# 3DOM-FBK/deep-image-matching

Measured on NVIDIA H100. Metric: image-pairs/sec (SuperPoint+LightGlue, 1024x1024, 2048 kpts), higher is better.
Workload: dtype f16 hi/lo split x3 MMA, f32 accumulate (fp32-class)

## Files before the change

deep-image-matching_b200/csrc/gemm.cuh:

```cuda
#pragma once
#include "common.cuh"
#include "sm90.cuh"

struct TileCoord {
  int m0;
  int n0;
  int b, y0, x0;
};

struct GemmArgs {
  int num_kb;
  int k_total;
  int M;
  int N;
  int cin_blocks;
  int H, W;
  int tiles_x, tiles_y;
  const __half *Ah, *Al, *Bh, *Bl;
  int lda, ldb;
};

constexpr int kTileM = 128;
constexpr int kGemmThreads = 12 * 32;
constexpr int kProducerRegs = 40, kConsumerRegs = 232;
constexpr int kScratchPitch = 32;
constexpr int kScratchFloats = 32 * kScratchPitch;
constexpr int kStgCols = 64, kStgPitch = kStgCols + 4;
constexpr int kStgFloats = 64 * kStgPitch;
constexpr int kStgBytes = 2 * kStgFloats * 4;
static_assert(4 * kScratchFloats <= kStgFloats, "functor scratch must fit in the staging buffer of a warpgroup");
constexpr int kConvTH = 8, kConvTW = 16;
template <int CONV>
struct ConvTile {
  static constexpr int TH = kConvTH, TW = kConvTW;
};

template <int CONV>
__device__ __forceinline__ TileCoord make_tile_coord(const GemmArgs& g, int t) {
  TileCoord tc;
  if (CONV == 1) {
    int per_img = g.tiles_x * g.tiles_y;
    tc.b = t / per_img;
    int rem = t - tc.b * per_img;
    tc.y0 = (rem / g.tiles_x) * ConvTile<CONV>::TH;
    tc.x0 = (rem % g.tiles_x) * ConvTile<CONV>::TW;
    tc.m0 = 0;
    tc.n0 = 0;
  } else {
    tc.m0 = t * kTileM;
    tc.n0 = 0;
    tc.b = tc.y0 = tc.x0 = 0;
  }
  return tc;
}

struct PersCfg {
  int sa, sb;
  int nkb_total;
  int smem_bytes;
};

template <int BN, bool SPLIT, int CONV>
struct PersGeom {
  static constexpr int kPl = SPLIT ? 2 : 1;
  static constexpr int kRowB = CONV == 3 ? 64 : 128;
  static constexpr int kABoxTx = CONV == 1 ? (kConvTH + 2) * kConvTW * 128 : kTileM * kRowB;
  static constexpr int kABox = (kABoxTx + 1023) / 1024 * 1024;
  static constexpr int kATx = kPl * kABoxTx;
  static constexpr int kAStage = kPl * kABox;
  static constexpr int kBPlane = BN * kRowB;
  static constexpr int kBTile = kPl * kBPlane;
  static constexpr int kBudget = 232448 - 1024 - 1024 - kStgBytes;
};

template <int BN, bool SPLIT, int CONV, bool RESB, class Epi>
__global__ void __launch_bounds__(kGemmThreads, 1)
tc_gemm_pers_kernel(const __grid_constant__ CUtensorMap tmAh, const __grid_constant__ CUtensorMap tmAl,
                    const __grid_constant__ CUtensorMap tmBh, const __grid_constant__ CUtensorMap tmBl, GemmArgs g, Epi epi,
                    int m_tiles, int n_tiles, int SA, int SB) {
  using G = PersGeom<BN, SPLIT, CONV>;
  using namespace sm90;
  static_assert(BN % kStgCols == 0, "BN must be a multiple of the staging width");
  extern __shared__ uint8_t smem_raw[];
  uint8_t* smem = smem_raw + ((1024u - (sm90::smem_u32(smem_raw) & 1023u)) & 1023u);
  constexpr bool ISCONV = CONV == 1;
  constexpr bool K32 = CONV == 3;
  constexpr int KB_COLS = K32 ? 32 : 64;
  constexpr int KSTEPS = K32 ? 2 : 4;
  constexpr uint32_t kLayout = K32 ? kLayoutSw64 : kLayoutSw128;
  constexpr uint32_t kSbo = 8 * G::kRowB;
  const int nkb = g.num_kb;
  uint8_t* sA = smem;
  uint8_t* sB = sA + SA * G::kAStage;
  const int nb_slots = RESB ? nkb : SB;
  uint64_t* fullA = reinterpret_cast<uint64_t*>(sB + nb_slots * G::kBTile);
  uint64_t* emptyA = fullA + SA;
  uint64_t* fullB = emptyA + SA;
  uint64_t* emptyB = fullB + nb_slots;
  float* staging = reinterpret_cast<float*>(reinterpret_cast<uint8_t*>(fullA) + 1024);

  const int warp = threadIdx.x >> 5, lane = threadIdx.x & 31;
  if (threadIdx.x == 0) {
    for (int s = 0; s < SA; ++s) {
      mbar_init(&fullA[s], 1);
      mbar_init(&emptyA[s], 8);
    }
    for (int s = 0; s < nb_slots; ++s) {
      mbar_init(&fullB[s], 1);
      mbar_init(&emptyB[s], 8);
    }
    fence_barrier_init();
  }
  __syncthreads();
  const int total = m_tiles * n_tiles;
  const int cinb = ISCONV ? g.cin_blocks : 1;
  const int outer_n = ISCONV ? 3 * cinb : nkb;
  constexpr int inner_n = ISCONV ? 3 : 1;
  auto kb_of = [&](int o, int in) { return ISCONV ? ((in * 3 + o / cinb) * cinb + (o % cinb)) : o; };

  auto tile_coord = [&](int w, int& n0) {
    const int mt = w / n_tiles, nt = w - mt * n_tiles;
    TileCoord tc = make_tile_coord<CONV>(g, mt);
    if (!ISCONV) tc.m0 = epi.m0_of(mt);
    n0 = nt * BN;
    tc.n0 = n0;
    return tc;
  };

  if (warp >= 8) {
    setmaxnreg_dec<kProducerRegs>();
    if (warp == 8) {
      if (elect_one()) {
        tma_prefetch_desc(&tmAh);
        tma_prefetch_desc(&tmBh);
        if (SPLIT) {
          tma_prefetch_desc(&tmAl);
          tma_prefetch_desc(&tmBl);
        }
      }
      __syncwarp();
      if (RESB && elect_one()) {
        const int nres = (static_cast<int>(blockIdx.x) % n_tiles) * BN;
        for (int kb = 0; kb < nkb; ++kb) {
          mbar_expect_tx(&fullB[kb], G::kBTile);
          tma_load_2d(sB + kb * G::kBTile, &tmBh, &fullB[kb], kb * KB_COLS, nres);
          if (SPLIT) tma_load_2d(sB + kb * G::kBTile + G::kBPlane, &tmBl, &fullB[kb], kb * KB_COLS, nres);
        }
      }
      __syncwarp();
      uint32_t itA = 0, itB = 0;
      for (int w = blockIdx.x; w < total; w += gridDim.x) {
        int n0;
        const TileCoord tc = tile_coord(w, n0);
        if (!epi.tile_active(tc)) continue;
        const int b_off = epi.b_row_offset(tc);
        const int outer = outer_n;
        if (elect_one()) {
          const int wp = w + 2 * static_cast<int>(gridDim.x);
          if (wp < total) {
            int n0p;
            const TileCoord tp = tile_coord(wp, n0p);
            if ((ISCONV || n0p == 0) && epi.tile_active(tp)) {
              for (int o = 0; o < outer; ++o) {
                if (ISCONV) {
                  const int dx = o / cinb, cb = o - dx * cinb;
                  if (dx != 1) continue;
                  tma_prefetch_4d(&tmAh, cb * 64, tp.x0 - 1, tp.y0 - 1, tp.b);
                  if (SPLIT) tma_prefetch_4d(&tmAl, cb * 64, tp.x0 - 1, tp.y0 - 1, tp.b);
                  tma_prefetch_4d(&tmAh, cb * 64, tp.x0 + 1, tp.y0 - 1, tp.b);
                  if (SPLIT) tma_prefetch_4d(&tmAl, cb * 64, tp.x0 + 1, tp.y0 - 1, tp.b);
                } else {
                  tma_prefetch_2d(&tmAh, o * KB_COLS, tp.m0);
                  if (SPLIT) tma_prefetch_2d(&tmAl, o * KB_COLS, tp.m0);
                }
              }
            }
          }
        }
        __syncwarp();
        for (int o = 0; o < outer; ++o) {
          const int s = itA % SA;
          mbar_wait(&emptyA[s], ((itA / SA) & 1) ^ 1);
          uint8_t* st = sA + s * G::kAStage;
          if (elect_one()) {
            mbar_expect_tx(&fullA[s], G::kATx);
            if (ISCONV) {
              const int dx = o / cinb, cb = o - dx * cinb;
              tma_load_4d(st, &tmAh, &fullA[s], cb * 64, tc.x0 + dx - 1, tc.y0 - 1, tc.b);
              if (SPLIT) tma_load_4d(st + G::kABox, &tmAl, &fullA[s], cb * 64, tc.x0 + dx - 1, tc.y0 - 1, tc.b);
            } else {
              tma_load_2d(st, &tmAh, &fullA[s], o * KB_COLS, tc.m0);
              if (SPLIT) tma_load_2d(st + G::kABox, &tmAl, &fullA[s], o * KB_COLS, tc.m0);
            }
          }
          __syncwarp();
          ++itA;
          if (!RESB) {
            for (int dy = 0; dy < inner_n; ++dy) {
              const int kb = kb_of(o, dy);
              const int sb = itB % SB;
              mbar_wait(&emptyB[sb], ((itB / SB) & 1) ^ 1);
              uint8_t* bt = sB + sb * G::kBTile;
              if (elect_one()) {
                mbar_expect_tx(&fullB[sb], G::kBTile);
                tma_load_2d(bt, &tmBh, &fullB[sb], kb * KB_COLS, n0 + b_off);
                if (SPLIT) tma_load_2d(bt + G::kBPlane, &tmBl, &fullB[sb], kb * KB_COLS, n0 + b_off);
              }
              __syncwarp();
              ++itB;
            }
          }
        }
      }
    }
  } else {
    setmaxnreg_inc<kConsumerRegs>();
    const int wg = warp >> 2, w4 = warp & 3;
    const uint32_t a_wg = static_cast<uint32_t>(wg * 64 * G::kRowB);
    float* stg = staging + wg * kStgFloats;
    uint32_t itA = 0, itB = 0;
    bool resb_ready = false;
    float acc[BN / 2];
    for (int w = blockIdx.x; w < total; w += gridDim.x) {
      int n0;
      const TileCoord tc = tile_coord(w, n0);
      if (!epi.tile_active(tc)) continue;
      const int outer = outer_n;
      for (int o = 0; o < outer; ++o) {
        const int s = itA % SA;
        mbar_wait(&fullA[s], (itA / SA) & 1);
        const uint32_t a_base = smem_u32(sA + s * G::kAStage) + a_wg;
        int sb0 = 0;
#pragma unroll
        for (int dy = 0; dy < inner_n; ++dy) {
          const int kb = kb_of(o, dy);
          uint32_t b_base;
          if (RESB) {
            if (!resb_ready) mbar_wait(&fullB[kb], 0);
            b_base = smem_u32(sB + kb * G::kBTile);
          } else {
            const int sb = (itB + dy) % SB;
            if (dy == 0) sb0 = sb;
            mbar_wait(&fullB[sb], ((itB + dy) / SB) & 1);
            b_base = smem_u32(sB + sb * G::kBTile);
          }
          const uint32_t a_tap = a_base + (ISCONV ? dy * (kConvTW * 128) : 0);
          const uint64_t a_h = make_sdesc(a_tap, kSbo, kLayout), a_l = make_sdesc(a_tap + G::kABox, kSbo, kLayout);
          const uint64_t b_h = make_sdesc(b_base, kSbo, kLayout), b_l = make_sdesc(b_base + G::kBPlane, kSbo, kLayout);
          wgmma_fence();
#pragma unroll
          for (int k16 = 0; k16 < KSTEPS; ++k16) {
            Wgmma<BN>::ss(acc, sdesc_advance_k(a_h, k16), sdesc_advance_k(b_h, k16), (o | dy | k16) != 0);
            if (SPLIT) {
              Wgmma<BN>::ss(acc, sdesc_advance_k(a_h, k16), sdesc_advance_k(b_l, k16), 1);
              Wgmma<BN>::ss(acc, sdesc_advance_k(a_l, k16), sdesc_advance_k(b_h, k16), 1);
            }
          }
        }
        wgmma_commit();
        wgmma_wait<0>();
        wgmma_fence_regs(acc);
        if (lane == 0) {
          mbar_arrive(&emptyA[s]);
          if (!RESB)
            for (int dy = 0; dy < inner_n; ++dy) mbar_arrive(&emptyB[(sb0 + dy) % SB]);
        }
        ++itA;
        if (!RESB) itB += inner_n;
      }
      resb_ready = true;
      const int rr = 32 * (w4 & 1) + lane, cq = 32 * (w4 >> 1);
#pragma unroll
      for (int c0 = 0; c0 < BN; c0 += kStgCols) {
        const int lr = 16 * w4 + (lane >> 2);
#pragma unroll
        for (int i = c0 / 8; i < (c0 + kStgCols) / 8; ++i) {
          const int col = 8 * i - c0 + 2 * (lane & 3);
          *reinterpret_cast<float2*>(stg + lr * kStgPitch + col) = make_float2(acc[4 * i], acc[4 * i + 1]);
          *reinterpret_cast<float2*>(stg + (lr + 8) * kStgPitch + col) = make_float2(acc[4 * i + 2], acc[4 * i + 3]);
        }
        named_bar_sync(1 + wg, 128);
        float v[32];
#pragma unroll
        for (int q = 0; q < 8; ++q) {
          const float4 x = *reinterpret_cast<const float4*>(stg + rr * kStgPitch + cq + 4 * q);
          v[4 * q] = x.x, v[4 * q + 1] = x.y, v[4 * q + 2] = x.z, v[4 * q + 3] = x.w;
        }
        named_bar_sync(1 + wg, 128);
        epi(tc, 64 * wg + rr, n0 + c0 + cq, v, stg + w4 * kScratchFloats);
        named_bar_sync(1 + wg, 128);
      }
    }
    if (RESB && !resb_ready)
      for (int kb = 0; kb < nkb; ++kb) mbar_wait(&fullB[kb], 0);
  }
}

template <int CONV>
__device__ __forceinline__ float simt_load_a(const GemmArgs& g, const TileCoord& tc, int row, int k) {
  size_t off;
  if (CONV == 1) {
    const int cin = g.cin_blocks * 64;
    const int tap = k / cin, c = k - tap * cin;
    const int dy = tap / 3, dx = tap - dy * 3;
    const int y = tc.y0 + row / ConvTile<CONV>::TW + dy - 1, x = tc.x0 + row % ConvTile<CONV>::TW + dx - 1;
    if (y < 0 || y >= g.H || x < 0 || x >= g.W) return 0.f;
    off = ((static_cast<size_t>(tc.b) * g.H + y) * g.W + x) * cin + c;
  } else {
    const int gm = tc.m0 + row;
    if (gm >= g.M) return 0.f;
    off = static_cast<size_t>(gm) * g.lda + k;
  }
  float v = __half2float(g.Ah[off]);
  if (g.Al) v += __half2float(g.Al[off]);
  return v;
}

template <int CONV, class Epi>
__global__ void __launch_bounds__(128) simt_gemm_kernel(GemmArgs g, Epi epi) {
  TileCoord tc = make_tile_coord<CONV>(g, blockIdx.x);
  if (CONV != 1) tc.m0 = epi.m0_of(blockIdx.x);
  tc.n0 = blockIdx.y * 32;
  if (!epi.tile_active(tc)) return;
  const int b_off = epi.b_row_offset(tc);
  __shared__ float As[128][33];
  __shared__ float Bs[32][33];
  __shared__ __align__(16) float scratchS[4 * kScratchFloats];
  const int t = threadIdx.x, n0 = blockIdx.y * 32;
  float acc[32];
#pragma unroll
  for (int j = 0; j < 32; ++j) acc[j] = 0.f;
  const int K = g.k_total ? g.k_total : g.num_kb * 64;
  for (int k0 = 0; k0 < K; k0 += 32) {
    const int kk = t & 31;
    for (int i = 0; i < 32; ++i) {
      const int row = i * 4 + (t >> 5);
      As[row][kk] = simt_load_a<CONV>(g, tc, row, k0 + kk);
    }
    for (int i = 0; i < 8; ++i) {
      const int nn = i * 4 + (t >> 5);
      float b = 0.f;
      if (n0 + nn < g.N) {
        const size_t off = static_cast<size_t>(n0 + nn + b_off) * g.ldb + k0 + kk;
        b = __half2float(g.Bh[off]);
        if (g.Bl) b += __half2float(g.Bl[off]);
      }
      Bs[nn][kk] = b;
    }
    __syncthreads();
#pragma unroll 4
    for (int k = 0; k < 32; ++k) {
      const float a = As[t][k];
#pragma unroll
      for (int j = 0; j < 32; ++j) acc[j] = fmaf(a, Bs[j][k], acc[j]);
    }
    __syncthreads();
  }
  epi(tc, t, n0, acc, scratchS + (t >> 5) * kScratchFloats);
}

struct TcOperands {
  CUtensorMap Ah, Al, Bh, Bl;
};

template <int BN, bool SPLIT, int CONV, bool RESB, class Epi>
int launch_pers(dimb_ctx* ctx, cudaStream_t st, const TcOperands& ops, const GemmArgs& g, const Epi& epi, int m_tiles, int n_tiles,
                const PersCfg& cfg, int grid) {
  auto kern = tc_gemm_pers_kernel<BN, SPLIT, CONV, RESB, Epi>;
  DIMB_TRY(dimb_func_smem(ctx, kern, cfg.smem_bytes));
  kern<<<grid, kGemmThreads, cfg.smem_bytes, st>>>(ops.Ah, ops.Al, ops.Bh, ops.Bl, g, epi, m_tiles, n_tiles, cfg.sa, cfg.sb);
  DIMB_LAUNCH_CHECK(ctx);
  return DIMB_OK;
}

template <int BN, bool SPLIT, int CONV>
PersCfg pers_config(int nkb, bool resb) {
  using G = PersGeom<BN, SPLIT, CONV>;
  PersCfg c{};
  c.nkb_total = nkb;
  int budget = G::kBudget;
  if (resb) {
    budget -= nkb * G::kBTile;
    c.sb = 0;
    c.sa = budget / G::kAStage;
  } else {
    const int per = CONV == 1 ? 3 : 1;
    const int unit = G::kAStage + per * G::kBTile;
    int n = budget / unit;
    if (n < 1) n = 1;
    c.sa = n;
    c.sb = per * n;
    while (c.sa * G::kAStage + (c.sb + 1) * G::kBTile <= budget) ++c.sb;
    while ((c.sa + 1) * G::kAStage + c.sb * G::kBTile <= budget) ++c.sa;
  }
  if (c.sa > 8) c.sa = 8;
  if (c.sb > 12) c.sb = 12;
  c.smem_bytes = c.sa * G::kAStage + (resb ? nkb : c.sb) * G::kBTile + 1024 + 1024 + kStgBytes;
  return c;
}

template <int BN, bool SPLIT, int CONV, class Epi>
int launch_pers_auto(dimb_ctx* ctx, cudaStream_t st, const TcOperands& ops, const GemmArgs& g, const Epi& epi, int m_tiles, int n_pad) {
  using G = PersGeom<BN, SPLIT, CONV>;
  const int n_tiles = n_pad / BN;
  const int total = m_tiles * n_tiles, grid = total < ctx->num_sms ? total : ctx->num_sms;
  const bool fits = Epi::kConstB && (G::kBudget - g.num_kb * G::kBTile) >= 2 * G::kAStage;
  int rgrid = grid;
  if (fits && grid % n_tiles != 0 && n_tiles <= grid) rgrid = grid / n_tiles * n_tiles;
  const bool resb = fits && (rgrid % n_tiles == 0) && rgrid * 8 >= grid * 7;
  if (resb)
    return launch_pers<BN, SPLIT, CONV, true, Epi>(ctx, st, ops, g, epi, m_tiles, n_tiles, pers_config<BN, SPLIT, CONV>(g.num_kb, true),
                                                   rgrid);
  return launch_pers<BN, SPLIT, CONV, false, Epi>(ctx, st, ops, g, epi, m_tiles, n_tiles, pers_config<BN, SPLIT, CONV>(g.num_kb, false),
                                                  grid);
}

template <int BN, int CONV, class Epi>
int launch_gemm(dimb_ctx* ctx, cudaStream_t st, const TcOperands& ops, GemmArgs g, const Epi& epi, int m_tiles, int n_pad,
                const char* tag = "gemm", int force_split = -1) {
  if (m_tiles <= 0) return DIMB_OK;
  ProfScope prof(ctx, st, tag);
  if (ctx->use_tc) {
    const bool exact = force_split < 0 ? ctx->precision == DIMB_PRECISION_EXACT : force_split != 0;
    if (exact) return launch_pers_auto<BN, true, CONV, Epi>(ctx, st, ops, g, epi, m_tiles, n_pad);
    return launch_pers_auto<BN, false, CONV, Epi>(ctx, st, ops, g, epi, m_tiles, n_pad);
  }
  if (force_split < 0 ? ctx->precision != DIMB_PRECISION_EXACT : force_split == 0) g.Al = g.Bl = nullptr;
  dim3 grid(m_tiles, n_pad / 32);
  simt_gemm_kernel<CONV, Epi><<<grid, 128, 0, st>>>(g, epi);
  DIMB_LAUNCH_CHECK(ctx);
  return DIMB_OK;
}

struct EpiBase {
  static constexpr bool kConstB = true;
  __device__ int m0_of(int t) const { return t * kTileM; }
  __device__ int b_row_offset(const TileCoord&) const { return 0; }
  __device__ bool tile_active(const TileCoord&) const { return true; }
};

__device__ __forceinline__ void warp_transpose32(const float (&v)[32], float* sc, float4 (&f)[8]) {
  const int lane = threadIdx.x & 31;
  float4* dst = reinterpret_cast<float4*>(sc + lane * kScratchPitch);
#pragma unroll
  for (int q = 0; q < 8; ++q) dst[q ^ (lane & 7)] = make_float4(v[4 * q], v[4 * q + 1], v[4 * q + 2], v[4 * q + 3]);
  __syncwarp();
#pragma unroll
  for (int it = 0; it < 8; ++it) {
    const int row = it * 4 + (lane >> 3);
    f[it] = *reinterpret_cast<const float4*>(sc + row * kScratchPitch + (((lane & 7) ^ (row & 7)) << 2));
  }
  __syncwarp();
}
__device__ __forceinline__ void store_split4(__half* hi, __half* lo, const float4& x) {
  __half2 h[2], l[2];
  split2_f32(x.x, x.y, h[0], l[0]);
  split2_f32(x.z, x.w, h[1], l[1]);
  *reinterpret_cast<uint2*>(hi) = *reinterpret_cast<const uint2*>(h);
  if (lo) *reinterpret_cast<uint2*>(lo) = *reinterpret_cast<const uint2*>(l);
}

__device__ __forceinline__ void store_half8(__half* dst, const __half (&h)[8]) {
  *reinterpret_cast<uint4*>(dst) = *reinterpret_cast<const uint4*>(h);
}

__device__ __forceinline__ void store_split32(__half* hi, __half* lo, const float (&v)[32]) {
#pragma unroll
  for (int q = 0; q < 4; ++q) {
    __half2 h[4], l[4];
#pragma unroll
    for (int j = 0; j < 4; ++j) split2_f32(v[q * 8 + 2 * j], v[q * 8 + 2 * j + 1], h[j], l[j]);
    *reinterpret_cast<uint4*>(hi + q * 8) = *reinterpret_cast<const uint4*>(h);
    if (lo) *reinterpret_cast<uint4*>(lo + q * 8) = *reinterpret_cast<const uint4*>(l);
  }
}

__device__ __forceinline__ void add_bias32(float (&v)[32], const float* __restrict__ bias, int n) {
  const float4* b4 = reinterpret_cast<const float4*>(bias + n);
#pragma unroll
  for (int q = 0; q < 8; ++q) {
    const float4 b = __ldg(b4 + q);
    v[4 * q] += b.x;
    v[4 * q + 1] += b.y;
    v[4 * q + 2] += b.z;
    v[4 * q + 3] += b.w;
  }
}

struct EpiStoreF32 : EpiBase {
  float* out;
  const float* bias;
  int ldc, n_valid, m_valid;
  float scale;
  __device__ void operator()(const TileCoord& tc, int r, int n, float (&v)[32], float* sc) const {
    const int lane = r & 31, col = n + (lane & 7) * 4;
    float4 b = make_float4(0.f, 0.f, 0.f, 0.f);
    if (bias && col + 3 < n_valid) b = __ldg(reinterpret_cast<const float4*>(bias + col));
    float4 f[8];
    warp_transpose32(v, sc, f);
#pragma unroll
    for (int it = 0; it < 8; ++it) {
      const int row = tc.m0 + (r & ~31) + it * 4 + (lane >> 3);
      if (row >= m_valid) continue;
      float* o = out + static_cast<size_t>(row) * ldc + col;
      if (col + 3 < n_valid && (ldc & 3) == 0) {
        *reinterpret_cast<float4*>(o) = make_float4((f[it].x + b.x) * scale, (f[it].y + b.y) * scale, (f[it].z + b.z) * scale,
                                                    (f[it].w + b.w) * scale);
      } else {
        const float e[4] = {f[it].x, f[it].y, f[it].z, f[it].w};
        for (int j = 0; j < 4; ++j)
          if (col + j < n_valid) o[j] = (e[j] + (bias ? bias[col + j] : 0.f)) * scale;
      }
    }
  }
};

struct EpiStoreSplit : EpiBase {
  __half *hi, *lo;
  const float* bias;
  int ldc, col_off, n_valid, m_valid;
  float scale;
  __device__ void operator()(const TileCoord& tc, int r, int n, float (&v)[32], float* sc) const {
    const int lane = r & 31, col = n + (lane & 7) * 4;
    const float4 b = (bias && n < n_valid) ? __ldg(reinterpret_cast<const float4*>(bias + col)) : make_float4(0.f, 0.f, 0.f, 0.f);
    float4 f[8];
    warp_transpose32(v, sc, f);
    if (n >= n_valid) return;
#pragma unroll
    for (int it = 0; it < 8; ++it) {
      const int row = tc.m0 + (r & ~31) + it * 4 + (lane >> 3);
      if (row >= m_valid) continue;
      const size_t off = static_cast<size_t>(row) * ldc + col_off + col;
      store_split4(hi + off, lo ? lo + off : nullptr,
                   make_float4((f[it].x + b.x) * scale, (f[it].y + b.y) * scale, (f[it].z + b.z) * scale, (f[it].w + b.w) * scale));
    }
  }
};
```

Measured before the change: 221.7.

## Pipeline consumer WGMMA per k-block with lagged stage release and deferred epilogue

The consumer now commits WGMMA groups per k-block and, for conv tiles, keeps one group in flight (wait<1>), releasing the previous A/B stages one step late. This lets the wait on the next TMA stage overlap with tensor-core work. When BN equals the staging width, the last epilogue chunk of a tile is deferred and run after the first MMA group of the next tile is issued, overlapping epilogue with MMA. The config also forces at least two A and two B stages when only one would fit by the unit rule. The cost is more complex barrier and release logic and extra live registers for the deferred chunk.

```diff
diff --git a/deep-image-matching_b200/csrc/gemm.cuh b/deep-image-matching_b200/csrc/gemm.cuh
--- a/deep-image-matching_b200/csrc/gemm.cuh
+++ b/deep-image-matching_b200/csrc/gemm.cuh
@@ -72,6 +72,23 @@
   static constexpr int kBTile = kPl * kBPlane;
   static constexpr int kBudget = 232448 - 1024 - 1024 - kStgBytes;
 };
+
+__device__ __forceinline__ void stage_chunk(const float* f, float* stg, float (&v)[32], int w4, int lane, int rr, int cq, int bar) {
+  const int lr = 16 * w4 + (lane >> 2);
+#pragma unroll
+  for (int i = 0; i < kStgCols / 8; ++i) {
+    const int col = 8 * i + 2 * (lane & 3);
+    *reinterpret_cast<float2*>(stg + lr * kStgPitch + col) = make_float2(f[4 * i], f[4 * i + 1]);
+    *reinterpret_cast<float2*>(stg + (lr + 8) * kStgPitch + col) = make_float2(f[4 * i + 2], f[4 * i + 3]);
+  }
+  sm90::named_bar_sync(bar, 128);
+#pragma unroll
+  for (int q = 0; q < 8; ++q) {
+    const float4 x = *reinterpret_cast<const float4*>(stg + rr * kStgPitch + cq + 4 * q);
+    v[4 * q] = x.x, v[4 * q + 1] = x.y, v[4 * q + 2] = x.z, v[4 * q + 3] = x.w;
+  }
+  sm90::named_bar_sync(bar, 128);
+}
 
 template <int BN, bool SPLIT, int CONV, bool RESB, class Epi>
 __global__ void __launch_bounds__(kGemmThreads, 1)
@@ -218,30 +235,54 @@
     const int wg = warp >> 2, w4 = warp & 3;
     const uint32_t a_wg = static_cast<uint32_t>(wg * 64 * G::kRowB);
     float* stg = staging + wg * kStgFloats;
+    const int rr = 32 * (w4 & 1) + lane, cq = 32 * (w4 >> 1);
     uint32_t itA = 0, itB = 0;
     bool resb_ready = false;
+    const bool lag = ISCONV && SA >= 2 && (RESB || SB >= 2);
     float acc[BN / 2];
+    constexpr bool kDefer = BN == kStgCols;
+    constexpr int kChunks = BN / kStgCols;
+    float v[32];
+    bool pending = false;
+    TileCoord ptc{};
+    int pn0 = 0;
+    auto run_deferred = [&]() {
+      epi(ptc, 64 * wg + rr, pn0 + BN - kStgCols + cq, v, stg + w4 * kScratchFloats);
+      named_bar_sync(1 + wg, 128);
+    };
     for (int w = blockIdx.x; w < total; w += gridDim.x) {
       int n0;
       const TileCoord tc = tile_coord(w, n0);
       if (!epi.tile_active(tc)) continue;
       const int outer = outer_n;
+      constexpr int kEpiDy = ISCONV ? 1 : 0;
+      const int epi_o = ISCONV || outer < 2 ? 0 : 1;
+      int prev_s = 0, prev_sb = 0;
       for (int o = 0; o < outer; ++o) {
         const int s = itA % SA;
-        mbar_wait(&fullA[s], (itA / SA) & 1);
         const uint32_t a_base = smem_u32(sA + s * G::kAStage) + a_wg;
-        int sb0 = 0;
 #pragma unroll
         for (int dy = 0; dy < inner_n; ++dy) {
           const int kb = kb_of(o, dy);
+          const int sb = RESB ? 0 : static_cast<int>(itB % SB);
+          const bool has_prev = lag && (o | dy) != 0;
+          bool released = false;
+          if (has_prev && !((dy != 0 || mbar_try_wait(&fullA[s], (itA / SA) & 1)) &&
+                            (RESB || mbar_try_wait(&fullB[sb], (itB / SB) & 1)))) {
+            wgmma_wait<0>();
+            if (lane == 0) {
+              if (!RESB) mbar_arrive(&emptyB[prev_sb]);
+              if (dy == 0) mbar_arrive(&emptyA[prev_s]);
+            }
+            released = true;
+          }
+          if (dy == 0) mbar_wait(&fullA[s], (itA / SA) & 1);
           uint32_t b_base;
           if (RESB) {
             if (!resb_ready) mbar_wait(&fullB[kb], 0);
             b_base = smem_u32(sB + kb * G::kBTile);
           } else {
-            const int sb = (itB + dy) % SB;
-            if (dy == 0) sb0 = sb;
-            mbar_wait(&fullB[sb], ((itB + dy) / SB) & 1);
+            mbar_wait(&fullB[sb], (itB / SB) & 1);
             b_base = smem_u32(sB + sb * G::kBTile);
           }
           const uint32_t a_tap = a_base + (ISCONV ? dy * (kConvTW * 128) : 0);
@@ -256,41 +297,52 @@
               Wgmma<BN>::ss(acc, sdesc_advance_k(a_l, k16), sdesc_advance_k(b_h, k16), 1);
             }
           }
+          wgmma_commit();
+          if (kDefer && dy == kEpiDy && o == epi_o && pending) {
+            run_deferred();
+            pending = false;
+          }
+          if (lag) {
+            wgmma_wait<1>();
+            if (has_prev && !released && lane == 0) {
+              if (!RESB) mbar_arrive(&emptyB[prev_sb]);
+              if (dy == 0) mbar_arrive(&emptyA[prev_s]);
+            }
+          } else {
+            wgmma_wait<0>();
+            if (lane == 0) {
+              if (!RESB) mbar_arrive(&emptyB[sb]);
+              if (dy == inner_n - 1) mbar_arrive(&emptyA[s]);
+            }
+          }
+          prev_sb = sb;
+          if (!RESB) ++itB;
         }
-        wgmma_commit();
-        wgmma_wait<0>();
-        wgmma_fence_regs(acc);
-        if (lane == 0) {
-          mbar_arrive(&emptyA[s]);
-          if (!RESB)
-            for (int dy = 0; dy < inner_n; ++dy) mbar_arrive(&emptyB[(sb0 + dy) % SB]);
+        prev_s = s;
+        ++itA;
+      }
+      wgmma_wait<0>();
+      wgmma_fence_regs(acc);
+      if (lag && lane == 0) {
+        if (!RESB) mbar_arrive(&emptyB[prev_sb]);
+        mbar_arrive(&emptyA[prev_s]);
+      }
+      resb_ready = true;
+#pragma unroll
+      for (int c = 0; c < kChunks; ++c) {
+        stage_chunk(acc + c * kStgCols / 2, stg, v, w4, lane, rr, cq, 1 + wg);
+        if (!kDefer || c < kChunks - 1) {
+          epi(tc, 64 * wg + rr, n0 + c * kStgCols + cq, v, stg + w4 * kScratchFloats);
+          named_bar_sync(1 + wg, 128);
         }
-        ++itA;
-        if (!RESB) itB += inner_n;
-      }
-      resb_ready = true;
-      const int rr = 32 * (w4 & 1) + lane, cq = 32 * (w4 >> 1);
-#pragma unroll
-      for (int c0 = 0; c0 < BN; c0 += kStgCols) {
-        const int lr = 16 * w4 + (lane >> 2);
-#pragma unroll
-        for (int i = c0 / 8; i < (c0 + kStgCols) / 8; ++i) {
-          const int col = 8 * i - c0 + 2 * (lane & 3);
-          *reinterpret_cast<float2*>(stg + lr * kStgPitch + col) = make_float2(acc[4 * i], acc[4 * i + 1]);
-          *reinterpret_cast<float2*>(stg + (lr + 8) * kStgPitch + col) = make_float2(acc[4 * i + 2], acc[4 * i + 3]);
-        }
-        named_bar_sync(1 + wg, 128);
-        float v[32];
-#pragma unroll
-        for (int q = 0; q < 8; ++q) {
-          const float4 x = *reinterpret_cast<const float4*>(stg + rr * kStgPitch + cq + 4 * q);
-          v[4 * q] = x.x, v[4 * q + 1] = x.y, v[4 * q + 2] = x.z, v[4 * q + 3] = x.w;
-        }
-        named_bar_sync(1 + wg, 128);
-        epi(tc, 64 * wg + rr, n0 + c0 + cq, v, stg + w4 * kScratchFloats);
-        named_bar_sync(1 + wg, 128);
-      }
-    }
+      }
+      if (kDefer) {
+        ptc = tc;
+        pn0 = n0;
+        pending = true;
+      }
+    }
+    if (pending) run_deferred();
     if (RESB && !resb_ready)
       for (int kb = 0; kb < nkb; ++kb) mbar_wait(&fullB[kb], 0);
   }
@@ -390,6 +442,10 @@
     if (n < 1) n = 1;
     c.sa = n;
     c.sb = per * n;
+    if (n == 1 && 2 * G::kAStage + 2 * G::kBTile <= budget) {
+      c.sa = 2;
+      c.sb = 2;
+    }
     while (c.sa * G::kAStage + (c.sb + 1) * G::kBTile <= budget) ++c.sb;
     while ((c.sa + 1) * G::kAStage + c.sb * G::kBTile <= budget) ++c.sa;
   }
```

Measured after the change: 227.9, median of 6. 1.03x the previous value.
